# ErikNatanael/knaster

Measured on AMD Instinct MI355X. Metric: UGen-samples/sec (voices x block_size x UGens / s), higher is better.
Workload: dtype f32

## Files before the change

knaster_amd/csrc/voice_bank.hpp:

```cpp
#pragma once

namespace {

template <typename F>
struct Bank final : knh_bank {
  typedef typename knh_dev::WordOf<F>::type W;
  const knh::KernelEntry* entry = nullptr;
  const knh::PipeEntry* pipe = nullptr;
  bool pipe_pair = false;
  const knh::WideEntry* wide = nullptr;
  int wide_waves = 0;
  bool interp = false;
  std::vector<knh_dev::InterpOp> h_prog;
  knh_dev::InterpOp* d_prog = nullptr;
  unsigned interp_sigs = 0, interp_out = 0;
  const knh::JitKernel* frame_jit = nullptr;
  uint32_t* d_sin_slots = nullptr;
  unsigned frame_vpw = 1, n_sin = 0;
  uint64_t env_ranks = 0;
  const knh::JitKernel* jit = nullptr;
  int pipeline_level = 1;
  std::string signature;
  const char* debug_signature() const override { return signature.c_str(); }
  uint32_t nv = 0;
// ... 380 lines not shown
      const unsigned n_cuts = partition_chain(signature, cuts);
      jit = knh::jit_pipe_kernel(signature.c_str(), cuts, n_cuts, sizeof(F) == 8, desc.allow_fma != 0, &why);
      jit_pipe = jit != nullptr;
      if (!jit) return fail(why.rfind("JIT_CRASH: ", 0) == 0 ? KNH_ERR_INTERNAL : KNH_ERR_UNSUPPORTED_CHAIN, "run-time fusion of chain '" + signature + "' (pipelined) failed: " + why);
    } else if (!entry && !interp) {
      std::string why;
      unsigned jw = !signature_is_dag(signature) && n_groups > jit_pipe_max ? (n_groups <= 1024 ? 4u : 8u) : 1u;
      if (const char* e = std::getenv("KNH_JIT_WAVES")) { const int v = std::atoi(e); if ((v == 1 || v == 4 || v == 8 || v == 16) && !signature_is_dag(signature)) jw = static_cast<unsigned>(v); }
      if (sizeof(F) == 8 && jw == 16) jw = 8;
      jit = knh::jit_voice_kernel(signature.c_str(), sizeof(F) == 8, desc.allow_fma != 0, &why, jw);
      if (!jit) return fail(why.rfind("JIT_CRASH: ", 0) == 0 ? KNH_ERR_INTERNAL : KNH_ERR_UNSUPPORTED_CHAIN, "run-time fusion of chain '" + signature + "' failed: " + why);
    }
    sample_rate = sr;
    block_size = bs;
    stride = (static_cast<long>(nv) + 63) / 64 * 64;
    f2pi = 16384.0 * 65536.0 * (1.0 / static_cast<double>(sr));
    const F sr_as_f32 = static_cast<F>(static_cast<float>(sr));

    std::vector<W> st(static_cast<size_t>(n_slots) * stride, W(0));
    std::vector<double> seg_rows;
    auto slot = [&](int s, uint32_t v) -> W& { return st[static_cast<size_t>(s) * stride + v]; };
    auto fw = [](F x) { return static_cast<W>(to_bits(x)); };
    shadow.assign(stages.size(), Shadow{});
    for (size_t si = 0; si < stages.size(); ++si) {
      const StageInfo& S = stages[si];
      const double* ca = ctor[si].data();
      Shadow& sh = shadow[si];
      for (uint32_t v = 0; v < nv; ++v) {
        const double* a = ca + static_cast<size_t>(v) * S.n_ctor;
        switch (S.kind) {
          case KNH_STAGE_SIN_WT: {
            if (v == 0) sh.a.resize(nv);
            F freq = static_cast<F>(a[0]);
            sh.a[v] = freq;
            slot(S.slot_base + 0, v) = 0;
            slot(S.slot_base + 1, v) = 0;
            slot(S.slot_base + 2, v) = sat_u32(static_cast<double>(freq) * f2pi);
          } break;
          case KNH_STAGE_SIN_NUMERIC: {
            F freq = static_cast<F>(a[0]);
            slot(S.slot_base + 0, v) = fw(F(0));
            slot(S.slot_base + 1, v) = fw(F(0));
            slot(S.slot_base + 2, v) = fw(freq / sr_as_f32);
          } break;
          case KNH_STAGE_SVF: {
            if (v == 0) { sh.a.resize(nv); sh.b.resize(nv); sh.c.resize(nv); sh.ty.resize(nv); }
            double tyd = a[0];
            uint32_t ty = (tyd >= 0 && tyd <= 8) ? static_cast<uint32_t>(tyd) : 0u;
            sh.ty[v] = static_cast<uint8_t>(ty);
            sh.a[v] = static_cast<F>(a[1]); sh.b[v] = static_cast<F>(a[2]); sh.c[v] = static_cast<F>(a[3]);
            F co[6];
            svf_coeffs<F>(ty, sh.a[v], sh.b[v], sh.c[v], sr_as_f32, co);
            slot(S.slot_base + 0, v) = fw(F(0));
            slot(S.slot_base + 1, v) = fw(F(0));
            for (int k = 0; k < 6; ++k) slot(S.slot_base + 2 + k, v) = fw(co[k]);
            if (S.n_slots == 12) {
              slot(S.slot_base + 8, v) = fw(sh.a[v]); slot(S.slot_base + 9, v) = fw(sh.b[v]); slot(S.slot_base + 10, v) = fw(sh.c[v]);
              slot(S.slot_base + 11, v) = ty;
            }
          } break;
          case KNH_STAGE_ONEPOLE_LPF:
          case KNH_STAGE_ONEPOLE_HPF: {
            F freq = S.kind == KNH_STAGE_ONEPOLE_LPF ? static_cast<F>(a[0]) : F(0);
            F f = freq / sr_as_f32;
            F b1 = std::exp(F(-2.0) * Consts<F>::PI * f);
            F a0 = F(1.0) - b1;
            slot(S.slot_base + 0, v) = fw(F(0));
            slot(S.slot_base + 1, v) = fw(a0);
            slot(S.slot_base + 2, v) = fw(b1);
          } break;
          case KNH_STAGE_MUL_ENV_ASR:
          case KNH_STAGE_MUL_ENV_AR: {
            if (v == 0) { sh.a.resize(nv); sh.b.resize(nv); }
            F atk = static_cast<F>(a[0]), rel = static_cast<F>(a[1]);
            sh.a[v] = atk; sh.b[v] = rel;
            F ar = atk == F(0) ? F(1) : F(1) / (atk * static_cast<F>(sr));
            F rr = rel == F(0) ? F(1) : F(1) / (rel * static_cast<F>(sr));
// ... 1313 lines not shown
```

knaster_amd/csrc/voice_chain.hpp:

```cpp
#pragma once
#include "voice_stages.hpp"

namespace knh_dev {

template <typename F, bool FMA, int BASE, typename... S> struct Chain;
template <typename F, bool FMA, int BASE>
struct Chain<F, FMA, BASE> {
  static constexpr int kSlots = BASE;
  static constexpr bool kUsesSine = false;
  static constexpr bool kPan = false;
  static constexpr u64 kParamBits = 0ull, kNopOkBits = 0ull;
  static constexpr bool kBinds = false;
  static constexpr bool kUsesRing = false;
  template <int T> __device__ __forceinline__ void tick_tile_sw(const Chain&, u32, u64, F (&)[T], const Ctx&, u32) {}
  __device__ __forceinline__ void pan_gains(F&, F&) const {}
  template <typename W> __device__ __forceinline__ void load(const W*, long) {}
  template <typename W> __device__ __forceinline__ void store(W*, long) const {}
  __device__ __forceinline__ F tick(F x, const Ctx&, u32) { return x; }
  template <int T> __device__ __forceinline__ void tick_tile(F (&)[T], const Ctx&, u32) {}
#ifdef KNH_DAG_STAMPS
  template <int T> __device__ __forceinline__ void tick_tile_stamped(F (&)[T], const Ctx&, u32, u64*, u64&) {}
#endif
  __device__ __forceinline__ void on_event(u32, u32, u64, u32) {}
  __device__ __forceinline__ bool last_env_stopped(bool dflt) const { return dflt; }
  __device__ __forceinline__ u32 collect_done(u32 acc) const { return acc; }
  __device__ __forceinline__ void reset_marks() {}
  __device__ __forceinline__ void begin_block(u32, const Ctx&) {}
};
template <typename F, bool FMA, int BASE, typename S0, typename... Rest>
struct Chain<F, FMA, BASE, S0, Rest...> {
  typedef Chain<F, FMA, BASE + S0::kSlots, Rest...> RestT;
  static constexpr int kSlots = RestT::kSlots;
  static constexpr bool kUsesSine = S0::kUsesSine || RestT::kUsesSine;
  static constexpr bool kPan = IsPan<S0>::value || RestT::kPan;
  static constexpr u64 kStageBits = BASE + S0::kSlots <= 64 ? (((u64)1 << S0::kSlots) - 1) << (BASE < 64 ? BASE : 0) : 0ull;
  static constexpr u64 kParamBits = (BASE + S0::kSlots <= 64 ? (u64)S0::kParamMask << (BASE < 64 ? BASE : 0) : 0ull) | RestT::kParamBits;
  static constexpr u64 kNopOkBits = ((S0::kParamMask != 0u || !S0::kHasSeg) && BASE < 64 ? (u64)1 << (BASE < 64 ? BASE : 0) : 0ull) | RestT::kNopOkBits;
  static constexpr bool kBinds = S0::kNeedsBind || RestT::kBinds;
  static constexpr bool kUsesRing = S0::kUsesRing || RestT::kUsesRing;
  typename S0::template Regs<F> r;
  u32 mark = 0xFFFFFFFFu;
  RestT rest;
  template <typename W> __device__ __forceinline__ void load(const W* s, long stride) {
    S0::template load<F, W>(r, s + (long)BASE * stride, stride);
    rest.load(s, stride);
  }
  template <typename W> __device__ __forceinline__ void store(W* s, long stride) const {
    S0::template store<F, W>(r, s + (long)BASE * stride, stride);
    rest.store(s, stride);
  }
  __device__ __forceinline__ F tick(F x, const Ctx& c, u32 frame) {
    x = S0::template tick<F, FMA>(r, x, c, frame, mark);
    return rest.tick(x, c, frame);
  }
  template <int T> __device__ __forceinline__ void tick_tile(F (&x)[T], const Ctx& c, u32 frame0) {
    S0::template tick_tile<F, FMA, T>(r, x, c, frame0, mark);
    rest.template tick_tile<T>(x, c, frame0);
  }
#ifdef KNH_DAG_STAMPS
  template <int T> __device__ __forceinline__ void tick_tile_stamped(F (&x)[T], const Ctx& c, u32 frame0, u64* acc, u64& t_prev) {
    S0::template tick_tile<F, FMA, T>(r, x, c, frame0, mark);
    asm volatile("" : "+v"(x[T - 1]) : : "memory");
    const u64 t = __builtin_amdgcn_s_memtime();
    acc[0] += t - t_prev;
    t_prev = t;
    rest.template tick_tile_stamped<T>(x, c, frame0, acc + 1, t_prev);
  }
#endif
  template <int T> __device__ __forceinline__ void tick_tile_sw(const Chain& cn, u32 sw, u64 touched, F (&x)[T], const Ctx& c, u32 frame0) {
    bool hit = false;
    if constexpr (S0::kParamMask != 0u) hit = __builtin_amdgcn_ballot_w64((touched & kStageBits) != 0ull) != 0;
    if (hit) {
#pragma unroll
      for (int j = 0; j < T; ++j) {
        S0::take_params(r, cn.r, (u32)j == sw);
        x[j] = S0::template tick<F, FMA>(r, x[j], c, frame0 + j, mark);
      }
    } else {
#pragma unroll
      for (int j = 0; j < T; ++j) x[j] = S0::template tick<F, FMA>(r, x[j], c, frame0 + j, mark);
// ... 1031 lines not shown
```

knaster_amd/csrc/voice_pipe.hpp:

```cpp
#pragma once
#include "voice_chain.hpp"

namespace knh_dev {

template <typename... S> struct Group {};
template <int K, typename... S> struct Fan {};

template <typename G> struct GroupInfo;
template <typename... S> struct GroupInfo<Group<S...>> {
  static constexpr int slots = (0 + ... + S::kSlots);
  static constexpr bool uses_sine = (false || ... || S::kUsesSine);
  static constexpr bool uses_ring = (false || ... || S::kUsesRing);
  static constexpr bool has_env = (false || ... || S::kIsEnv);
  static constexpr bool pan = (false || ... || IsPan<S>::value);
  static constexpr int fan_for(int) { return 1; }
};
template <int K, typename... S> struct GroupInfo<Fan<K, S...>> {
  static constexpr int slots = (0 + ... + S::kSlots);
  static constexpr bool uses_sine = (false || ... || S::kUsesSine);
  static constexpr bool uses_ring = false;
  static constexpr bool has_env = false;
  static constexpr bool pan = false;
  static constexpr int fan_for(int T) { return K * 8 <= T ? K : (T >= 8 ? T / 8 : 1); }
  static_assert(((S::kMutableMask == 0u) && ...), "a Fan group's stages keep no state");
// ... 10 lines not shown
template <typename F> struct PipeTile {
  static constexpr int value = sizeof(F) == 4 ? 32 : 16;
  static constexpr int big = 2 * value;
};

template <typename F, int TILE> struct EdgeLayout {
  static constexpr int T = TILE;
  static constexpr int VW = 16 / (int)sizeof(F);
  static constexpr int stride = T + VW;
  static constexpr int tile = 64 * stride;
  typedef F Vec __attribute__((ext_vector_type(16 / sizeof(F))));
};
enum { PIPE_MIXER = 0, PIPE_FOLD = 1, PIPE_INPLACE = 2 };
template <int MODE, int NG> struct EdgeMap {
  static_assert(MODE != PIPE_INPLACE || NG >= 2, "an in-place last group reads an edge");
  static constexpr int tiles = MODE == PIPE_MIXER ? NG * 2 : NG * 2 - 1;
  static __device__ __forceinline__ int out_tile(int I, int g) {
    if (MODE == PIPE_FOLD && I == NG - 1) return I * 2;
    if (MODE == PIPE_INPLACE && I >= NG - 2) return (NG - 2) * 2 + g % 3;
    return I * 2 + (g & 1);
  }
  static __device__ __forceinline__ int in_tile(int I, int g) { return I > 0 ? out_tile(I - 1, g) : 0; }
  static __device__ __forceinline__ int mixer_tile(int g) { return out_tile(NG - 1, g); }
};
__device__ __forceinline__ void pipe_barrier() {
  __builtin_amdgcn_fence(__ATOMIC_RELEASE, "workgroup");
  __builtin_amdgcn_s_barrier();
  __builtin_amdgcn_fence(__ATOMIC_ACQUIRE, "workgroup");
}

template <typename F> struct PipeShared {
  float* sine;
  F* edge;
  const Event* ev_lds;
  u32 ev_lds_first, ev_lds_n;
  u32* res_slot;
  u32* res_marks;
  Event* ev_stage;
  u32 ev_cap, n_threads;
  __attribute__((address_space(3))) char* ring_tile_of[4];
};

template <typename F, bool FMA, int T, bool PAN>
__device__ __forceinline__ void pipe_fold_tile(const F* tile, const VoiceKernelArgs<F>& a, int lane, u32 wave_global, u32 n_waves_total,
                                               int blk, u32 n0, u32 len, u32 v0, u32 nv, u32 res_tile = 0u, u32 res_epoch = 0u);

// ... 93 lines not shown
    chain.reset_marks();
    const ResStaged st = res_stage_events(a.res, call, sh.ev_stage, sh.ev_cap, v0, nv, (u32)(wave_all * 64 + lane), sh.n_threads);
    ev_staged = st.count != 0u;
    ev_lds_first = st.first;
    ev_ranged = call.has_events && call.n_ranges != 0u;
    if (ev_ranged) { evs = nullptr; ev_i = 0; ev_end = call.n_ranges; }
  }
  if (!ev_ranged) {
    ev_i = 0; ev_end = 0;
    if (evs) {
      if (resident) { ev_i = *reinterpret_cast<const volatile u32*>(evs + voice); ev_end = *reinterpret_cast<const volatile u32*>(evs + voice + 1); }
      else { ev_i = evs[voice]; ev_end = evs[voice + 1]; }
    }
  }
  nxt.frame = 0xFFFFFFFFu; next_frame = 0xFFFFFFFFu;
  take_next();
  base = 0;

  const u32 n_frames = fend - fbeg;
  const int tpb = (int)((n_frames + T - 1) / T);
  const int n_tiles = tpb * (int)a.n_blocks;
  const int n_steps = n_tiles + NG - (MODE == PIPE_FOLD ? 1 : 0);
  const u32 n_waves_total = (a.n_voices + 63u) / 64u;
  int blk = 0, ti = 0;
#ifdef KNH_DAG_STAMPS
  u64 busy = 0, busy_in = 0, busy_out = 0, busy_tick = 0, busy_fold = 0;
#endif
  for (int s = 0; s < n_steps; ++s) {
    const int g = s - I;
    if (g >= 0 && g < n_tiles) {
#ifdef KNH_DAG_STAMPS
      const u64 t0 = __builtin_amdgcn_s_memtime();
#endif
      F x[TW];
      if (I > 0) {
        typedef typename EdgeLayout<F, T>::Vec Vec;
        constexpr int VW = EdgeLayout<F, T>::VW;
        const Vec* in = reinterpret_cast<const Vec*>(sh.edge + (long)Map::in_tile(I, g) * EdgeLayout<F, T>::tile +
                                                     (long)lane * EdgeLayout<F, T>::stride + fo);
#pragma unroll
        for (int j = 0; j < TW / VW; ++j) {
          const Vec v = in[j];
#pragma unroll
          for (int k = 0; k < VW; ++k) x[j * VW + k] = v[k];
        }
      } else {
#pragma unroll
        for (int j = 0; j < TW; ++j) x[j] = (F)0;
      }
      if (ti == 0) {
        ctx.input_block = reinterpret_cast<const F*>(a.input) + (long)blk * a.in_channels * a.block_size;
        chain.begin_block(fbeg, ctx);
      }
      const u32 n_tile = fbeg + (u32)ti * T;
      const u32 m_tile = fend - n_tile < (u32)T ? fend - n_tile : (u32)T;
      const u32 n = n_tile + fo;
      const u32 m = m_tile > fo ? (m_tile - fo < (u32)TW ? m_tile - fo : (u32)TW) : 0u;
      apply_events_upto(base + n);
      const bool ev_inside = next_frame < base + n + TW;
#if defined(KNH_DAG_STAMPS) || defined(KNH_TILE_FENCES)
      asm volatile("s_waitcnt lgkmcnt(0)" ::: "memory");
#endif
#ifdef KNH_DAG_STAMPS
      const u64 t1 = __builtin_amdgcn_s_memtime();
      busy_in += t1 - t0;
#endif
      {
        typedef typename EdgeLayout<F, T>::Vec Vec;
        constexpr int VW = EdgeLayout<F, T>::VW;
        F* out_tile = sh.edge + (long)Map::out_tile(I, g) * EdgeLayout<F, T>::tile;
        F* out_row = out_tile + (long)lane * EdgeLayout<F, T>::stride + fo;
        if (__builtin_expect(m == (u32)TW && !__builtin_amdgcn_ballot_w64(ev_inside), 1)) {
          chain.template tick_tile<TW>(x, ctx, n);
#ifdef KNH_DAG_STAMPS
          asm volatile("" ::: "memory");
          busy_tick += __builtin_amdgcn_s_memtime() - t1;
#endif
          Vec* out = reinterpret_cast<Vec*>(out_row);
#pragma unroll
          for (int j = 0; j < TW / VW; ++j) {
            Vec v;
#pragma unroll
            for (int k = 0; k < VW; ++k) v[k] = x[j * VW + k];
            out[j] = v;
          }
#ifdef KNH_AB_NO_SW
        } else if (false && [&]() -> bool {
#else
        } else if (m == (u32)TW && ChainT::kParamBits != 0ull && !ChainT::kBinds && [&]() -> bool {
#endif
          ChainT cn = chain;
          const u32 sv_i = ev_i;
          const Event sv_nxt = nxt;
          const u32 sv_next_frame = next_frame;
          const u32 tile_end = base + n + (u32)TW;
          u32 sw = (u32)TW;
          u64 touched = 0ull;
          bool bad = false;
          while (next_frame < tile_end) {
            const u32 op = nxt.slot_op >> 24, slot = nxt.slot_op & 0xFFFFFFu, code = op & 0x7Fu;
            if (slot >= SLOT_LO && slot < SLOT_HI) {
              const u32 rel = nxt.frame - (base + n);
              if (sw == (u32)TW) sw = rel;
              bad = bad || sw != rel || slot >= 64u ||
                    !((code == EV_SET && ((ChainT::kParamBits >> (slot & 63u)) & 1ull)) || (code == EV_NOP && ((ChainT::kNopOkBits >> (slot & 63u)) & 1ull)));
              if (!bad) {
                cn.on_event(op, slot, nxt.bits, nxt.frame - base);
                touched |= 1ull << (slot & 63u);
                if (live && code == EV_SET) a.state[(long)slot * a.stride + voice] = (W)nxt.bits;
              }
            }
            ++ev_i;
            take_next();
          }
          if (__builtin_amdgcn_ballot_w64(bad) != 0) {
            ev_i = sv_i;
            nxt = sv_nxt;
            next_frame = sv_next_frame;
            return false;
          }
          const F* in_row = sh.edge + (long)Map::in_tile(I, g) * EdgeLayout<F, T>::tile + (long)lane * EdgeLayout<F, T>::stride + fo;
          for (u32 j0 = 0; j0 < (u32)TW; j0 += 8u) {
            F sub[8];
            if (I > 0) {
#pragma unroll
              for (int q = 0; q < 8 / VW; ++q) {
                const Vec v = reinterpret_cast<const Vec*>(in_row + j0)[q];
#pragma unroll
                for (int k = 0; k < VW; ++k) sub[q * VW + k] = v[k];
              }
            } else {
#pragma unroll
              for (int k = 0; k < 8; ++k) sub[k] = (F)0;
            }
            chain.template tick_tile_sw<8>(cn, sw - j0, touched, sub, ctx, n + j0);
#pragma unroll
            for (int q = 0; q < 8 / VW; ++q) {
              Vec v;
#pragma unroll
              for (int k = 0; k < VW; ++k) v[k] = sub[q * VW + k];
              reinterpret_cast<Vec*>(out_row + j0)[q] = v;
            }
          }
          return true;
        }()) {
        } else {
          const F* in_row = sh.edge + (long)Map::in_tile(I, g) * EdgeLayout<F, T>::tile + (long)lane * EdgeLayout<F, T>::stride + fo;
          for (u32 j0 = 0; j0 < m; j0 += 8u) {
            const u32 cnt = m - j0 < 8u ? m - j0 : 8u;
            F sub[8];
            if (I > 0) {
#pragma unroll
              for (int q = 0; q < 8 / VW; ++q) {
                const Vec v = reinterpret_cast<const Vec*>(in_row + j0)[q];
#pragma unroll
                for (int k = 0; k < VW; ++k) sub[q * VW + k] = v[k];
              }
            } else {
#pragma unroll
              for (int k = 0; k < 8; ++k) sub[k] = (F)0;
            }
#pragma unroll
            for (int k = 0; k < 8; ++k) {
              if ((u32)k < cnt) {
                apply_events_upto(base + n + j0 + (u32)k);
                sub[k] = chain.tick(sub[k], ctx, n + j0 + (u32)k);
              }
            }
#pragma unroll
            for (int q = 0; q < 8 / VW; ++q) {
              Vec v;
#pragma unroll
              for (int k = 0; k < VW; ++k) v[k] = sub[q * VW + k];
              reinterpret_cast<Vec*>(out_row + j0)[q] = v;
            }
          }
        }
        if constexpr (GroupInfo<G>::pan) {
          F gl = (F)0, gr = (F)0;
          chain.pan_gains(gl, gr);
          out_row[T] = gl;
          out_row[T + 1] = gr;
        }
#ifdef KNH_DAG_STAMPS
        asm volatile("s_waitcnt lgkmcnt(0)" ::: "memory");
        const u64 tf0 = __builtin_amdgcn_s_memtime();
#endif
        if constexpr (FOLDS) pipe_fold_tile<F, FMA, T, GroupInfo<G>::pan>(out_tile, a, lane, wave_global, n_waves_total, blk, n_tile, m_tile, v0, nv);
#ifdef KNH_DAG_STAMPS
        asm volatile("s_waitcnt lgkmcnt(0)" ::: "memory");
        busy_fold += __builtin_amdgcn_s_memtime() - tf0;
#endif
      }
#if defined(KNH_DAG_STAMPS) || defined(KNH_TILE_FENCES)
      asm volatile("" ::: "memory");
#endif
#ifdef KNH_DAG_STAMPS
      const u64 t2 = __builtin_amdgcn_s_memtime();
#endif
      if (++ti == tpb) {
        apply_events_upto(base + fend);
        ti = 0;
        ++blk;
        base += a.block_size;
        if (resident) {
          sh.res_marks[wave_all * 64 + lane] = chain.collect_done(0xFFFFFFFFu);
          if (GroupInfo<G>::has_env && I == LAST_ENV) sh.res_marks[15 * 64 + lane] = live && !chain.last_env_stopped(false) ? 1u : 0u;
        }
      }
#if defined(KNH_DAG_STAMPS) || defined(KNH_TILE_FENCES)
      asm volatile("s_waitcnt lgkmcnt(0)" ::: "memory");
#endif
#ifdef KNH_DAG_STAMPS
      const u64 t3 = __builtin_amdgcn_s_memtime();
      busy += t3 - t0;
      busy_out += t3 - t2;
#endif
    }
    pipe_barrier();
  }
#ifdef KNH_DAG_STAMPS
  if (wave_global == 0u && lane == 0) {
    const u64 d = (u64)(n_tiles > 0 ? n_tiles : 1);
    a.flags[4 + I] = (u32)(busy / d);
    if (8 + 2 * I + 1 < 16) { a.flags[8 + 2 * I] = (u32)(busy_in / d); a.flags[9 + 2 * I] = (u32)(busy_out / d); }
    if (FOLDS) { a.flags[14] = (u32)(busy_tick / d); a.flags[15] = (u32)(busy_fold / d); }
    else if (MODE != PIPE_FOLD && I == 1) { a.flags[14] = (u32)(busy_tick / d); a.flags[15] = (u32)((busy - busy_in - busy_out - busy_tick) / d); }
  }
#endif
  done_frame = chain.collect_done(0xFFFFFFFFu);
  if (!resident) break;
  }
  if (live) chain.store(a.state + voice, a.stride);
  if (!resident && GroupInfo<G>::has_env && I == LAST_ENV) {
    const bool running = live && !chain.last_env_stopped(false);
    const u64 br = __builtin_amdgcn_ballot_w64(running);
    if (lane == 0 && br) atomicAdd(&a.flags[1], (u32)__builtin_popcountll(br));
  }
  return done_frame;
}

template <typename F, bool FMA, int T, bool PAN>
__device__ __forceinline__ void pipe_fold_tile(const F* tile, const VoiceKernelArgs<F>& a, int lane, u32 wave_global, u32 n_waves_total,
// ... 31 lines not shown
}

template <typename F, bool FMA, int T, int MODE, int NG, bool PAN, int CHAINW, bool HAS_ENV>
__device__ __forceinline__ void pipe_run_mixer(const PipeShared<F>& sh, const VoiceKernelArgs<F>& a, int lane, u32 wave_global,
                                               u32 v0, u32 nv, int wave_all) {
  u32 fbeg = a.frame_begin, fend = a.frame_end;
  const bool resident = a.res.bell != nullptr;
  u32 res_expect = a.res.first_epoch;
  const u32 n_waves_total = (a.n_voices + 63u) / 64u;
  for (;;) {
  ResCall call;
  call.epoch = 0u;
  if (resident) {
    call = res_wait(a.res, res_expect, sh.res_slot, wave_all, lane);
    if (call.leave) break;
    res_expect = (res_expect + 1u) & (u32)RES_EPOCH_MASK;
    fbeg = call.frame_begin;
    fend = call.frame_end;
    (void)res_stage_events(a.res, call, sh.ev_stage, sh.ev_cap, v0, nv, (u32)(wave_all * 64 + lane), sh.n_threads);
  }
  const u32 n_frames = fend - fbeg;
  const int tpb = (int)((n_frames + T - 1) / T);
  const int n_tiles = tpb * (int)a.n_blocks;
  const int n_steps = n_tiles + NG;
  int blk = 0, ti = 0;
#ifdef KNH_DAG_STAMPS
  u64 busy = 0;
#endif
  for (int s = 0; s < n_steps; ++s) {
    const int g = s - NG;
    if (g >= 0 && g < n_tiles) {
#ifdef KNH_DAG_STAMPS
      const u64 t0 = __builtin_amdgcn_s_memtime();
#endif
      const u32 rel = (u32)ti * T;
      const u32 len = n_frames - rel < (u32)T ? n_frames - rel : (u32)T;
      const F* tile = sh.edge + (long)EdgeMap<MODE, NG>::mixer_tile(g) * EdgeLayout<F, T>::tile;
      pipe_fold_tile<F, FMA, T, PAN>(tile, a, lane, wave_global, n_waves_total, blk, fbeg + rel, len, v0, nv, (u32)g, call.epoch);
      if (resident && g == n_tiles - 1) {
        u32 n_done = 0u, n_run = 0u;
        if (HAS_ENV) {
          u32 d = 0xFFFFFFFFu;
#pragma unroll
          for (int w = 0; w < CHAINW; ++w) d = sh.res_marks[w * 64 + lane] != 0xFFFFFFFFu ? sh.res_marks[w * 64 + lane] : d;
          const bool live = (u32)lane < nv;
          if (live) a.done_frames[v0 + lane] = d;
          n_done = (u32)__builtin_popcountll(__builtin_amdgcn_ballot_w64(live && d != 0xFFFFFFFFu));
          n_run = (u32)__builtin_popcountll(__builtin_amdgcn_ballot_w64(live && sh.res_marks[15 * 64 + lane] != 0u));
        }
        if (lane == 0) res_put(a.res.wg_flags + wave_global, n_done | (n_run << 8), res_tag(call.epoch, 255u));
      }
      if (++ti == tpb) { ti = 0; ++blk; }
#ifdef KNH_DAG_STAMPS
      asm volatile("s_waitcnt vmcnt(0) lgkmcnt(0)" ::: "memory");
      busy += __builtin_amdgcn_s_memtime() - t0;
#endif
    }
    if (resident) asm volatile("s_waitcnt lgkmcnt(0)\n\ts_barrier" ::: "memory");
    else pipe_barrier();
  }
#ifdef KNH_DAG_STAMPS
  if (wave_global == 0u && lane == 0) a.flags[4 + NG] = (u32)(busy / (u64)(n_tiles > 0 ? n_tiles : 1));
#endif
  if (!resident) break;
  }
}

template <typename F, bool FMA, int T, int MODE, int NG, int I, int BASE, int W0, int LAST_ENV, typename G, typename... Rest>
__device__ __forceinline__ u32 pipe_dispatch(int wave, const PipeShared<F>& sh, const VoiceKernelArgs<F>& a, int lane, u32 wave_global, u32 v0, u32 nv, int wave_all) {
  constexpr int KF = GroupInfo<G>::fan_for(T);
  if (wave >= W0 && wave < W0 + KF) return pipe_run_group<F, FMA, T, MODE, NG, I, BASE, LAST_ENV, G>(sh, a, lane, wave_global, v0, nv, wave - W0, wave_all);
  if constexpr (sizeof...(Rest) > 0)
    return pipe_dispatch<F, FMA, T, MODE, NG, I + 1, BASE + GroupInfo<G>::slots, W0 + KF, LAST_ENV, Rest...>(wave, sh, a, lane, wave_global, v0, nv, wave_all);
  return 0xFFFFFFFFu;
}
template <int T, int MODE, typename... Gs> struct PipeWaves {
  static constexpr int chain = (0 + ... + GroupInfo<Gs>::fan_for(T));
  static constexpr int value = chain + (MODE == PIPE_FOLD ? 0 : 1);
};

template <int I, typename... Gs> struct LastEnv;
template <int I> struct LastEnv<I> { static constexpr int value = -1; };
// ... 117 lines not shown
```

knaster_amd/csrc/voice_stages.hpp:

```cpp
#pragma once

extern "C" __device__ float __ocml_sin_f32(float);
extern "C" __device__ double __ocml_sin_f64(double);
extern "C" __device__ float __ocml_cos_f32(float);
extern "C" __device__ double __ocml_cos_f64(double);
extern "C" __device__ float __ocml_pow_f32(float, float);
extern "C" __device__ double __ocml_pow_f64(double, double);
extern "C" __device__ float __ocml_tan_f32(float);
extern "C" __device__ double __ocml_tan_f64(double);
extern "C" __device__ float __ocml_exp_f32(float);
extern "C" __device__ double __ocml_exp_f64(double);
extern "C" __device__ float __ocml_sqrt_f32(float);
extern "C" __device__ double __ocml_sqrt_f64(double);

namespace knh_dev {

typedef unsigned int u32;
typedef unsigned long long u64;

template <typename F> struct WordOf;
template <> struct WordOf<float> { typedef u32 type; };
template <> struct WordOf<double> { typedef u64 type; };

template <typename F> __device__ __forceinline__ F word_to_f(typename WordOf<F>::type w);
// ... 3 lines not shown
__device__ __forceinline__ u64 f_to_word(double f) { return __builtin_bit_cast(u64, f); }

template <bool FMA> __device__ __forceinline__ float mad(float a, float b, float c) {
  if constexpr (FMA) return __builtin_fmaf(a, b, c);
  else return a * b + c;
}
template <bool FMA> __device__ __forceinline__ double mad(double a, double b, double c) {
  if constexpr (FMA) return __builtin_fma(a, b, c);
  else return a * b + c;
}

__device__ __forceinline__ u32 sat_u32(double v) {
  u32 r;
  asm("v_cvt_u32_f64 %0, %1" : "=v"(r) : "v"(v));
  return r;
}

struct StageDefaults {
  static constexpr u32 kParamMask = 0u;
  template <typename R> static __device__ __forceinline__ void take_params(R&, const R&, bool) {}
  static constexpr bool kBinary = false;
  static constexpr int kArParam = -1;
  static constexpr bool kUsesRing = false;
};
template <typename S, int P> struct ArP : S {
  static constexpr int kArParam = P;
};

enum { EV_SET = 0, EV_ENV_ASR_RELEASE = 1, EV_NOP = 2, EV_SEGENV_STOP = 3, EV_ALLPASS_DELAY = 4, EV_SPLIT = 0x80  };

struct Event {
  u32 frame;
  u32 slot_op;
  u64 bits;
};

struct Ctx {
  const float* sine;
  double f2pi;
  const double* seg_table;
  u32 seg_max;
  void* delay_ring;
  u32 delay_stride;
  const void* buffer;
  const void* input_block;
  u32 in_stride;
// ... 838 lines not shown
      "v_pk_mul_f32 v[102:103], v[116:117], v[100:101] op_sel_hi:[1,0]\n\t"      \
      "v_pk_mul_f32 v[104:105], v[118:119], v[114:115] op_sel_hi:[1,0]\n\t"      \
      "v_add_f32 v103, v101, v103\n\t"                                       \
      "v_pk_add_f32 v[106:107], v[102:103], v[104:105]\n\t"                  \
      "v_mul_f32 v112, v122, %[x" #K "]\n\t"                                 \
      "v_pk_fma_f32 v[100:101], v[106:107], 2.0, v[100:101] op_sel_hi:[1,0,1] neg_lo:[0,0,1] neg_hi:[0,0,1]\n\t"    \
      "v_pk_mul_f32 v[108:109], v[120:121], v[106:107]\n\t"                  \
      KNH_SVF_WAIT                                                                                                     \
      "v_add_f32 v112, v112, v108\n\t"                                       \
      "v_add_f32 %[y" #K "], v112, v109\n\t"
#pragma unroll
    for (int j = 0; j < T; j += 8) {
      float y0, y1, y2, y3, y4, y5, y6, y7;
      asm volatile(KNH_SVF_STEP(0) KNH_SVF_STEP(1) KNH_SVF_STEP(2) KNH_SVF_STEP(3) KNH_SVF_STEP(4) KNH_SVF_STEP(5) KNH_SVF_STEP(6) KNH_SVF_STEP(7)
                   : [y0] "=&v"(y0), [y1] "=&v"(y1), [y2] "=&v"(y2), [y3] "=&v"(y3), [y4] "=&v"(y4), [y5] "=&v"(y5),
                     [y6] "=&v"(y6), [y7] "=&v"(y7), "+{v100}"(ic1), "+{v101}"(ic2)
                   : [x0] "v"(x[j]), [x1] "v"(x[j + 1]), [x2] "v"(x[j + 2]), [x3] "v"(x[j + 3]), [x4] "v"(x[j + 4]),
                     [x5] "v"(x[j + 5]), [x6] "v"(x[j + 6]), [x7] "v"(x[j + 7]), "{v116}"(a1), "{v117}"(a2), "{v118}"(a2b), "{v119}"(a3),
                     "{v120}"(m1), "{v121}"(m2), "{v122}"(m0)
                   : "v102", "v103", "v104", "v105", "v106", "v107", "v108", "v109", "v112", "v114", "v115");
      x[j] = y0; x[j + 1] = y1; x[j + 2] = y2; x[j + 3] = y3; x[j + 4] = y4; x[j + 5] = y5; x[j + 6] = y6; x[j + 7] = y7;
    }
#undef KNH_SVF_STEP
    r.ic1 = ic1; r.ic2 = ic2;
  }
  template <typename F> static __device__ __forceinline__ bool low_pass(const Regs<F>& r) {
    typedef typename WordOf<F>::type W;
    const W neg0 = (W)1 << (sizeof(F) * 8 - 1);
    const bool mine = r.nl == 0 && f_to_word(r.ic2) != neg0;
    return __builtin_amdgcn_ballot_w64(!mine) == 0;
  }
  template <int T>
  static __device__ __forceinline__ void tick_tile_low(Regs<float>& r, float (&x)[T]) {
    static_assert(T % 8 == 0, "the filter tile is unrolled in blocks of eight samples");
    float ic1 = r.ic1, ic2 = r.ic2;
    const float a1 = r.a1, a2 = r.a2, a2b = r.a2, a3 = r.a3;
#define KNH_SVF_LOW(K)                                                                                             \
      "v_sub_f32 v114, %[x" #K "], v101\n\t"                                 \
      "v_pk_mul_f32 v[102:103], v[116:117], v[100:101] op_sel_hi:[1,0]\n\t"      \
      "v_pk_mul_f32 v[104:105], v[118:119], v[114:115] op_sel_hi:[1,0]\n\t"      \
      "v_add_f32 v103, v101, v103\n\t"                                       \
      "v_pk_add_f32 v[106:107], v[102:103], v[104:105]\n\t"                  \
      KNH_SVF_WAIT                                                                                                     \
      "v_fma_f32 %[y" #K "], 0, v106, v107\n\t"                              \
      "v_pk_fma_f32 v[100:101], v[106:107], 2.0, v[100:101] op_sel_hi:[1,0,1] neg_lo:[0,0,1] neg_hi:[0,0,1]\n\t"    \
      KNH_SVF_WAIT
#pragma unroll
    for (int j = 0; j < T; j += 8) {
      float y0, y1, y2, y3, y4, y5, y6, y7;
      asm volatile(KNH_SVF_LOW(0) KNH_SVF_LOW(1) KNH_SVF_LOW(2) KNH_SVF_LOW(3) KNH_SVF_LOW(4) KNH_SVF_LOW(5) KNH_SVF_LOW(6) KNH_SVF_LOW(7)
                   : [y0] "=&v"(y0), [y1] "=&v"(y1), [y2] "=&v"(y2), [y3] "=&v"(y3), [y4] "=&v"(y4), [y5] "=&v"(y5),
                     [y6] "=&v"(y6), [y7] "=&v"(y7), "+{v100}"(ic1), "+{v101}"(ic2)
                   : [x0] "v"(x[j]), [x1] "v"(x[j + 1]), [x2] "v"(x[j + 2]), [x3] "v"(x[j + 3]), [x4] "v"(x[j + 4]),
                     [x5] "v"(x[j + 5]), [x6] "v"(x[j + 6]), [x7] "v"(x[j + 7]), "{v116}"(a1), "{v117}"(a2), "{v118}"(a2b), "{v119}"(a3)
                   : "v102", "v103", "v104", "v105", "v106", "v107", "v114", "v115");
      x[j] = y0; x[j + 1] = y1; x[j + 2] = y2; x[j + 3] = y3; x[j + 4] = y4; x[j + 5] = y5; x[j + 6] = y6; x[j + 7] = y7;
    }
#undef KNH_SVF_LOW
    r.ic1 = ic1; r.ic2 = ic2;
  }
  template <int T>
  static __device__ __forceinline__ void tick_tile_low_f64(Regs<double>& r, double (&x)[T]) {
    double ic1 = r.ic1, ic2 = r.ic2;
    const double a1 = r.a1, a2 = r.a2, a3 = r.a3;
    double v1p = 0.0, v2p = 0.0;
#define KNH_STEP(stmt) stmt; __builtin_amdgcn_sched_barrier(0)
#pragma unroll
    for (int j = 0; j < T; ++j) {
      KNH_STEP(const double v3 = x[j] - ic2);
      KNH_STEP(const double p2 = a2 * ic1);
      KNH_STEP(const double p1 = a1 * ic1);
      KNH_STEP(const double q2 = a3 * v3);
      KNH_STEP(const double q1 = a2 * v3);
      KNH_STEP(const double t = ic2 + p2);
      if (j > 0) { KNH_STEP(x[j - 1] = __builtin_fma(0.0, v1p, v2p)); }
      KNH_STEP(const double v2 = t + q2);
      KNH_STEP(const double v1 = p1 + q1);
      KNH_STEP(ic2 = __builtin_fma(2.0, v2, -ic2));
      KNH_STEP(ic1 = __builtin_fma(2.0, v1, -ic1));
      v1p = v1; v2p = v2;
    }
    x[T - 1] = __builtin_fma(0.0, v1p, v2p);
// ... 10 lines not shown
    for (int j = 0; j < T; ++j) {
      double o1 = 0.0, o2 = 0.0, s = 0.0;
      KNH_STEP(const double v3 = x[j] - ic2);
      KNH_STEP(const double p1 = a1 * ic1);
      KNH_STEP(const double p2 = a2 * ic1);
      if (j > 0) { KNH_STEP(o1 = m1 * v1p); }
      KNH_STEP(const double q1 = a2 * v3);
      KNH_STEP(const double q2 = a3 * v3);
      KNH_STEP(const double t = ic2 + p2);
      if (j > 0) { KNH_STEP(o2 = m2 * v2p); }
      KNH_STEP(const double v1 = p1 + q1);
      KNH_STEP(const double v2 = t + q2);
      if (j > 0) { KNH_STEP(s = o0p + o1); }
      KNH_STEP(ic1 = __builtin_fma(2.0, v1, -ic1));
      KNH_STEP(ic2 = __builtin_fma(2.0, v2, -ic2));
      KNH_STEP(const double o0 = m0 * x[j]);
      if (j > 0) { KNH_STEP(x[j - 1] = s + o2); }
      v1p = v1; v2p = v2; o0p = o0;
    }
    x[T - 1] = (o0p + m1 * v1p) + m2 * v2p;
#undef KNH_STEP
    r.ic1 = ic1; r.ic2 = ic2;
  }
  template <typename F, bool FMA, int T>
  static __device__ __forceinline__ void tick_tile(Regs<F>& r, F (&x)[T], const Ctx& c, u32 frame0, u32& done_frame) {
    if constexpr (sizeof(F) == 4 && !FMA) {
      if (low_pass(r)) tick_tile_low<T>(r, x); else tick_tile_packed<T>(r, x);
    } else if constexpr (sizeof(F) == 8 && !FMA) {
      if (low_pass(r)) tick_tile_low_f64<T>(r, x); else tick_tile_f64<T>(r, x);
    } else {
#pragma unroll
      for (int j = 0; j < T; ++j) x[j] = tick<F, FMA>(r, x[j], c, frame0 + j, done_frame);
    }
  }
  template <typename F>
  static __device__ __forceinline__ void on_event(Regs<F>& r, u32 op, u32 rel, u64 bits, u32 ) {
    if ((op & 0x7Fu) != EV_SET) return;
    F v = word_to_f<F>((typename WordOf<F>::type)bits);
    r.ic1 = rel == 0 ? v : r.ic1; r.ic2 = rel == 1 ? v : r.ic2; r.a1 = rel == 2 ? v : r.a1; r.a2 = rel == 3 ? v : r.a2;
    r.a3 = rel == 4 ? v : r.a3; r.m0 = rel == 5 ? v : r.m0; r.m1 = rel == 6 ? v : r.m1; r.m2 = rel >= 7 ? v : r.m2;
    note_mix(r);
  }
};

static __device__ __forceinline__ float dev_pow(float a, float b) { return __ocml_pow_f32(a, b); }
static __device__ __forceinline__ double dev_pow(double a, double b) { return __ocml_pow_f64(a, b); }
struct SvfP : Svf {
  static constexpr int kSlots = 12;
  static constexpr u32 kParamMask = 0u;
  template <typename F> struct Regs : Svf::Regs<F> { F cutoff, q, gain; u32 ty; };
  template <typename F, typename W>
  static __device__ __forceinline__ void load(Regs<F>& r, const W* s, long st) {
    Svf::load<F, W>(r, s, st);
    r.cutoff = word_to_f<F>(s[8 * st]); r.q = word_to_f<F>(s[9 * st]); r.gain = word_to_f<F>(s[10 * st]); r.ty = (u32)s[11 * st];
  }
  template <typename F, typename W>
  static __device__ __forceinline__ void store(const Regs<F>& r, W* s, long st) {
    Svf::store<F, W>(r, s, st);
    s[2 * st] = f_to_word(r.a1); s[3 * st] = f_to_word(r.a2); s[4 * st] = f_to_word(r.a3);
    s[5 * st] = f_to_word(r.m0); s[6 * st] = f_to_word(r.m1); s[7 * st] = f_to_word(r.m2);
    s[8 * st] = f_to_word(r.cutoff); s[9 * st] = f_to_word(r.q); s[10 * st] = f_to_word(r.gain);
  }
  static __device__ __forceinline__ float tan_f(float v) { return __ocml_tan_f32(v); }
  static __device__ __forceinline__ double tan_f(double v) { return __ocml_tan_f64(v); }
  static __device__ __forceinline__ float sqrt_f(float v) { return __ocml_sqrt_f32(v); }
  static __device__ __forceinline__ double sqrt_f(double v) { return __ocml_sqrt_f64(v); }
  template <typename F>
  static __device__ __forceinline__ void set_coeffs(Regs<F>& r, const Ctx& c) {
    const F one = (F)1, sr = (F)(float)c.sample_rate;
    F g = tan_f(((F)3.14159265358979323846 * r.cutoff) / sr);
    F k = one / r.q;
    F m0 = (F)0, m1 = (F)0, m2 = (F)0, amp = (F)0;
// ... 978 lines not shown
```

Measured before the change: 2924 billion.

## Run event-free tile streaks in pipe kernel with hoisted SVF mode check

Restructures the pipelined voice kernel loop from a per-step dispatch into per-block loops. An inner fast path processes consecutive full tiles without events, using incrementally advanced edge tile indices instead of recomputing the tile map each step. A RunPrep mechanism evaluates the SVF low-pass mode check once per run rather than once per tile, and the mixer loop gets a similar incremental tile index. It also adds odd pinned-register inline asm for the SVF state writeback and a debug env toggle that seeds -0.0 into SVF state, which may constrain register allocation.

```diff
diff --git a/knaster_amd/csrc/voice_bank.hpp b/knaster_amd/csrc/voice_bank.hpp
--- a/knaster_amd/csrc/voice_bank.hpp
+++ b/knaster_amd/csrc/voice_bank.hpp
@@ -426,6 +426,8 @@
     auto slot = [&](int s, uint32_t v) -> W& { return st[static_cast<size_t>(s) * stride + v]; };
     auto fw = [](F x) { return static_cast<W>(to_bits(x)); };
     shadow.assign(stages.size(), Shadow{});
+    const char* const neg0_env = std::getenv("KNH_DEBUG_SVF_IC2_NEG0");
+    const bool svf_ic2_neg0 = neg0_env && neg0_env[0] == '1';
     for (size_t si = 0; si < stages.size(); ++si) {
       const StageInfo& S = stages[si];
       const double* ca = ctor[si].data();
@@ -456,7 +458,7 @@
             F co[6];
             svf_coeffs<F>(ty, sh.a[v], sh.b[v], sh.c[v], sr_as_f32, co);
             slot(S.slot_base + 0, v) = fw(F(0));
-            slot(S.slot_base + 1, v) = fw(F(0));
+            slot(S.slot_base + 1, v) = fw(svf_ic2_neg0 && v % 3 == 0 ? F(-0.0) : F(0));
             for (int k = 0; k < 6; ++k) slot(S.slot_base + 2 + k, v) = fw(co[k]);
             if (S.n_slots == 12) {
               slot(S.slot_base + 8, v) = fw(sh.a[v]); slot(S.slot_base + 9, v) = fw(sh.b[v]); slot(S.slot_base + 10, v) = fw(sh.c[v]);
diff --git a/knaster_amd/csrc/voice_chain.hpp b/knaster_amd/csrc/voice_chain.hpp
--- a/knaster_amd/csrc/voice_chain.hpp
+++ b/knaster_amd/csrc/voice_chain.hpp
@@ -18,6 +18,9 @@
   template <typename W> __device__ __forceinline__ void store(W*, long) const {}
   __device__ __forceinline__ F tick(F x, const Ctx&, u32) { return x; }
   template <int T> __device__ __forceinline__ void tick_tile(F (&)[T], const Ctx&, u32) {}
+  struct RunPrep {};
+  __device__ __forceinline__ RunPrep prepare_run() const { return RunPrep(); }
+  template <int T> __device__ __forceinline__ void tick_tile_run(F (&)[T], const Ctx&, u32, const RunPrep&) {}
 #ifdef KNH_DAG_STAMPS
   template <int T> __device__ __forceinline__ void tick_tile_stamped(F (&)[T], const Ctx&, u32, u64*, u64&) {}
 #endif
@@ -56,6 +59,19 @@
   template <int T> __device__ __forceinline__ void tick_tile(F (&x)[T], const Ctx& c, u32 frame0) {
     S0::template tick_tile<F, FMA, T>(r, x, c, frame0, mark);
     rest.template tick_tile<T>(x, c, frame0);
+  }
+  struct RunPrep { bool mine; typename RestT::RunPrep rest; };
+  __device__ __forceinline__ RunPrep prepare_run() const {
+    RunPrep p;
+    if constexpr (S0::kHasRunPrep) p.mine = S0::template prepare_run<F>(r);
+    else p.mine = false;
+    p.rest = rest.prepare_run();
+    return p;
+  }
+  template <int T> __device__ __forceinline__ void tick_tile_run(F (&x)[T], const Ctx& c, u32 frame0, const RunPrep& p) {
+    if constexpr (S0::kHasRunPrep) S0::template tick_tile_prepared<F, FMA, T>(r, x, c, frame0, mark, p.mine);
+    else S0::template tick_tile<F, FMA, T>(r, x, c, frame0, mark);
+    rest.template tick_tile_run<T>(x, c, frame0, p.rest);
   }
 #ifdef KNH_DAG_STAMPS
   template <int T> __device__ __forceinline__ void tick_tile_stamped(F (&x)[T], const Ctx& c, u32 frame0, u64* acc, u64& t_prev) {
diff --git a/knaster_amd/csrc/voice_pipe.hpp b/knaster_amd/csrc/voice_pipe.hpp
--- a/knaster_amd/csrc/voice_pipe.hpp
+++ b/knaster_amd/csrc/voice_pipe.hpp
@@ -56,6 +56,13 @@
   }
   static __device__ __forceinline__ int in_tile(int I, int g) { return I > 0 ? out_tile(I - 1, g) : 0; }
   static __device__ __forceinline__ int mixer_tile(int g) { return out_tile(NG - 1, g); }
+  static __device__ __forceinline__ int next_out(int I, int t) {
+    if (MODE == PIPE_FOLD && I == NG - 1) return t;
+    if (MODE == PIPE_INPLACE && I >= NG - 2) return t == (NG - 2) * 2 + 2 ? (NG - 2) * 2 : t + 1;
+    return t ^ 1;
+  }
+  static __device__ __forceinline__ int next_in(int I, int t) { return I > 0 ? next_out(I - 1, t) : 0; }
+  static __device__ __forceinline__ int next_mixer(int t) { return next_out(NG - 1, t); }
 };
 __device__ __forceinline__ void pipe_barrier() {
   __builtin_amdgcn_fence(__ATOMIC_RELEASE, "workgroup");
@@ -195,60 +202,61 @@
   const int n_tiles = tpb * (int)a.n_blocks;
   const int n_steps = n_tiles + NG - (MODE == PIPE_FOLD ? 1 : 0);
   const u32 n_waves_total = (a.n_voices + 63u) / 64u;
-  int blk = 0, ti = 0;
+  const int full = n_frames >= fo + (u32)TW ? (int)((n_frames - fo - (u32)TW) / (u32)T) + 1 : 0;
+  int in_t = Map::in_tile(I, 0), out_t = Map::out_tile(I, 0);
 #ifdef KNH_DAG_STAMPS
   u64 busy = 0, busy_in = 0, busy_out = 0, busy_tick = 0, busy_fold = 0;
 #endif
-  for (int s = 0; s < n_steps; ++s) {
-    const int g = s - I;
-    if (g >= 0 && g < n_tiles) {
+  for (int s = 0; s < I; ++s) pipe_barrier();
+  for (int blk = 0, ti = 0; blk < (tpb > 0 ? (int)a.n_blocks : 0); ++blk) {
+    ctx.input_block = reinterpret_cast<const F*>(a.input) + (long)blk * a.in_channels * a.block_size;
+    chain.begin_block(fbeg, ctx);
+    for (ti = 0;;) {
+      typedef typename EdgeLayout<F, T>::Vec Vec;
+      constexpr int VW = EdgeLayout<F, T>::VW;
 #ifdef KNH_DAG_STAMPS
       const u64 t0 = __builtin_amdgcn_s_memtime();
 #endif
-      F x[TW];
-      if (I > 0) {
-        typedef typename EdgeLayout<F, T>::Vec Vec;
-        constexpr int VW = EdgeLayout<F, T>::VW;
-        const Vec* in = reinterpret_cast<const Vec*>(sh.edge + (long)Map::in_tile(I, g) * EdgeLayout<F, T>::tile +
-                                                     (long)lane * EdgeLayout<F, T>::stride + fo);
-#pragma unroll
-        for (int j = 0; j < TW / VW; ++j) {
-          const Vec v = in[j];
-#pragma unroll
-          for (int k = 0; k < VW; ++k) x[j * VW + k] = v[k];
-        }
-      } else {
-#pragma unroll
-        for (int j = 0; j < TW; ++j) x[j] = (F)0;
-      }
-      if (ti == 0) {
-        ctx.input_block = reinterpret_cast<const F*>(a.input) + (long)blk * a.in_channels * a.block_size;
-        chain.begin_block(fbeg, ctx);
-      }
       const u32 n_tile = fbeg + (u32)ti * T;
-      const u32 m_tile = fend - n_tile < (u32)T ? fend - n_tile : (u32)T;
       const u32 n = n_tile + fo;
-      const u32 m = m_tile > fo ? (m_tile - fo < (u32)TW ? m_tile - fo : (u32)TW) : 0u;
       apply_events_upto(base + n);
       const bool ev_inside = next_frame < base + n + TW;
+      bool step_open = true;
+      if (__builtin_expect(ti < full && !__builtin_amdgcn_ballot_w64(ev_inside), 1)) {
+        const typename ChainT::RunPrep prep = chain.prepare_run();
+        u32 nq = n;
+        for (;;) {
+#ifdef KNH_DAG_STAMPS
+          const u64 q0 = __builtin_amdgcn_s_memtime();
+#endif
+          F x[TW];
+          if (I > 0) {
+            const Vec* in = reinterpret_cast<const Vec*>(sh.edge + (long)in_t * EdgeLayout<F, T>::tile + (long)lane * EdgeLayout<F, T>::stride + fo);
+#pragma unroll
+            for (int j = 0; j < TW / VW; ++j) {
+              const Vec v = in[j];
+#pragma unroll
+              for (int k = 0; k < VW; ++k) x[j * VW + k] = v[k];
+            }
+          } else {
+#pragma unroll
+            for (int j = 0; j < TW; ++j) x[j] = (F)0;
+          }
 #if defined(KNH_DAG_STAMPS) || defined(KNH_TILE_FENCES)
-      asm volatile("s_waitcnt lgkmcnt(0)" ::: "memory");
-#endif
-#ifdef KNH_DAG_STAMPS
-      const u64 t1 = __builtin_amdgcn_s_memtime();
-      busy_in += t1 - t0;
-#endif
-      {
-        typedef typename EdgeLayout<F, T>::Vec Vec;
-        constexpr int VW = EdgeLayout<F, T>::VW;
-        F* out_tile = sh.edge + (long)Map::out_tile(I, g) * EdgeLayout<F, T>::tile;
-        F* out_row = out_tile + (long)lane * EdgeLayout<F, T>::stride + fo;
-        if (__builtin_expect(m == (u32)TW && !__builtin_amdgcn_ballot_w64(ev_inside), 1)) {
-          chain.template tick_tile<TW>(x, ctx, n);
+          asm volatile("s_waitcnt lgkmcnt(0)" ::: "memory");
+#endif
+#ifdef KNH_DAG_STAMPS
+          const u64 q1 = __builtin_amdgcn_s_memtime();
+          busy_in += q1 - q0;
+#endif
+          chain.template tick_tile_run<TW>(x, ctx, nq, prep);
 #ifdef KNH_DAG_STAMPS
           asm volatile("" ::: "memory");
-          busy_tick += __builtin_amdgcn_s_memtime() - t1;
-#endif
+          const u64 q2 = __builtin_amdgcn_s_memtime();
+          busy_tick += q2 - q1;
+#endif
+          F* const out_tile = sh.edge + (long)out_t * EdgeLayout<F, T>::tile;
+          F* const out_row = out_tile + (long)lane * EdgeLayout<F, T>::stride + fo;
           Vec* out = reinterpret_cast<Vec*>(out_row);
 #pragma unroll
           for (int j = 0; j < TW / VW; ++j) {
@@ -257,10 +265,48 @@
             for (int k = 0; k < VW; ++k) v[k] = x[j * VW + k];
             out[j] = v;
           }
+          if constexpr (GroupInfo<G>::pan) {
+            F gl = (F)0, gr = (F)0;
+            chain.pan_gains(gl, gr);
+            out_row[T] = gl;
+            out_row[T + 1] = gr;
+          }
+#ifdef KNH_DAG_STAMPS
+          asm volatile("s_waitcnt lgkmcnt(0)" ::: "memory");
+          const u64 qf = __builtin_amdgcn_s_memtime();
+#endif
+          if constexpr (FOLDS) pipe_fold_tile<F, FMA, T, GroupInfo<G>::pan>(out_tile, a, lane, wave_global, n_waves_total, blk, nq, (u32)T, v0, nv);
+#ifdef KNH_DAG_STAMPS
+          asm volatile("s_waitcnt lgkmcnt(0)" ::: "memory");
+          const u64 qe = __builtin_amdgcn_s_memtime();
+          busy_fold += qe - qf;
+#endif
+          in_t = Map::next_in(I, in_t);
+          out_t = Map::next_out(I, out_t);
+          nq += (u32)T;
+          ++ti;
+#if defined(KNH_DAG_STAMPS) || defined(KNH_TILE_FENCES)
+          asm volatile("s_waitcnt lgkmcnt(0)" ::: "memory");
+#endif
+#ifdef KNH_DAG_STAMPS
+          const u64 q3 = __builtin_amdgcn_s_memtime();
+          busy_out += q3 - qe;
+          busy += q3 - q0;
+#endif
+          if (ti >= full) break;
+          pipe_barrier();
+          if (__builtin_amdgcn_ballot_w64(next_frame < base + nq + TW)) { step_open = false; break; }
+        }
+      } else {
+        const u32 m_tile = fend - n_tile < (u32)T ? fend - n_tile : (u32)T;
+        const u32 m = m_tile > fo ? (m_tile - fo < (u32)TW ? m_tile - fo : (u32)TW) : 0u;
+        F* const out_tile = sh.edge + (long)out_t * EdgeLayout<F, T>::tile;
+        F* const out_row = out_tile + (long)lane * EdgeLayout<F, T>::stride + fo;
+        const F* const in_row = sh.edge + (long)in_t * EdgeLayout<F, T>::tile + (long)lane * EdgeLayout<F, T>::stride + fo;
 #ifdef KNH_AB_NO_SW
-        } else if (false && [&]() -> bool {
+        if (false && [&]() -> bool {
 #else
-        } else if (m == (u32)TW && ChainT::kParamBits != 0ull && !ChainT::kBinds && [&]() -> bool {
+        if (m == (u32)TW && ChainT::kParamBits != 0ull && !ChainT::kBinds && [&]() -> bool {
 #endif
           ChainT cn = chain;
           const u32 sv_i = ev_i;
@@ -292,7 +338,6 @@
             next_frame = sv_next_frame;
             return false;
           }
-          const F* in_row = sh.edge + (long)Map::in_tile(I, g) * EdgeLayout<F, T>::tile + (long)lane * EdgeLayout<F, T>::stride + fo;
           for (u32 j0 = 0; j0 < (u32)TW; j0 += 8u) {
             F sub[8];
             if (I > 0) {
@@ -318,7 +363,6 @@
           return true;
         }()) {
         } else {
-          const F* in_row = sh.edge + (long)Map::in_tile(I, g) * EdgeLayout<F, T>::tile + (long)lane * EdgeLayout<F, T>::stride + fo;
           for (u32 j0 = 0; j0 < m; j0 += 8u) {
             const u32 cnt = m - j0 < 8u ? m - j0 : 8u;
             F sub[8];
@@ -360,38 +404,33 @@
         const u64 tf0 = __builtin_amdgcn_s_memtime();
 #endif
         if constexpr (FOLDS) pipe_fold_tile<F, FMA, T, GroupInfo<G>::pan>(out_tile, a, lane, wave_global, n_waves_total, blk, n_tile, m_tile, v0, nv);
+        in_t = Map::next_in(I, in_t);
+        out_t = Map::next_out(I, out_t);
+        ++ti;
 #ifdef KNH_DAG_STAMPS
         asm volatile("s_waitcnt lgkmcnt(0)" ::: "memory");
-        busy_fold += __builtin_amdgcn_s_memtime() - tf0;
+        const u64 t3 = __builtin_amdgcn_s_memtime();
+        busy_fold += t3 - tf0;
+        busy += t3 - t0;
 #endif
       }
-#if defined(KNH_DAG_STAMPS) || defined(KNH_TILE_FENCES)
-      asm volatile("" ::: "memory");
-#endif
-#ifdef KNH_DAG_STAMPS
-      const u64 t2 = __builtin_amdgcn_s_memtime();
-#endif
-      if (++ti == tpb) {
+      if (ti == tpb) {
         apply_events_upto(base + fend);
-        ti = 0;
-        ++blk;
         base += a.block_size;
         if (resident) {
           sh.res_marks[wave_all * 64 + lane] = chain.collect_done(0xFFFFFFFFu);
           if (GroupInfo<G>::has_env && I == LAST_ENV) sh.res_marks[15 * 64 + lane] = live && !chain.last_env_stopped(false) ? 1u : 0u;
         }
+#if defined(KNH_DAG_STAMPS) || defined(KNH_TILE_FENCES)
+        asm volatile("s_waitcnt lgkmcnt(0)" ::: "memory");
+#endif
+        pipe_barrier();
+        break;
       }
-#if defined(KNH_DAG_STAMPS) || defined(KNH_TILE_FENCES)
-      asm volatile("s_waitcnt lgkmcnt(0)" ::: "memory");
-#endif
-#ifdef KNH_DAG_STAMPS
-      const u64 t3 = __builtin_amdgcn_s_memtime();
-      busy += t3 - t0;
-      busy_out += t3 - t2;
-#endif
-    }
-    pipe_barrier();
-  }
+      if (step_open) pipe_barrier();
+    }
+  }
+  for (int s = I + n_tiles; s < n_steps; ++s) pipe_barrier();
 #ifdef KNH_DAG_STAMPS
   if (wave_global == 0u && lane == 0) {
     const u64 d = (u64)(n_tiles > 0 ? n_tiles : 1);
@@ -469,20 +508,23 @@
   const u32 n_frames = fend - fbeg;
   const int tpb = (int)((n_frames + T - 1) / T);
   const int n_tiles = tpb * (int)a.n_blocks;
-  const int n_steps = n_tiles + NG;
-  int blk = 0, ti = 0;
 #ifdef KNH_DAG_STAMPS
   u64 busy = 0;
 #endif
-  for (int s = 0; s < n_steps; ++s) {
-    const int g = s - NG;
-    if (g >= 0 && g < n_tiles) {
+  auto step_barrier = [&]() {
+    if (resident) asm volatile("s_waitcnt lgkmcnt(0)\n\ts_barrier" ::: "memory");
+    else pipe_barrier();
+  };
+  for (int s = 0; s < NG; ++s) step_barrier();
+  int mix_t = EdgeMap<MODE, NG>::mixer_tile(0);
+  int g = 0;
+  for (int blk = 0; blk < (tpb > 0 ? (int)a.n_blocks : 0); ++blk) {
+    for (u32 rel = 0; rel < n_frames; rel += (u32)T) {
 #ifdef KNH_DAG_STAMPS
       const u64 t0 = __builtin_amdgcn_s_memtime();
 #endif
-      const u32 rel = (u32)ti * T;
       const u32 len = n_frames - rel < (u32)T ? n_frames - rel : (u32)T;
-      const F* tile = sh.edge + (long)EdgeMap<MODE, NG>::mixer_tile(g) * EdgeLayout<F, T>::tile;
+      const F* tile = sh.edge + (long)mix_t * EdgeLayout<F, T>::tile;
       pipe_fold_tile<F, FMA, T, PAN>(tile, a, lane, wave_global, n_waves_total, blk, fbeg + rel, len, v0, nv, (u32)g, call.epoch);
       if (resident && g == n_tiles - 1) {
         u32 n_done = 0u, n_run = 0u;
@@ -497,14 +539,14 @@
         }
         if (lane == 0) res_put(a.res.wg_flags + wave_global, n_done | (n_run << 8), res_tag(call.epoch, 255u));
       }
-      if (++ti == tpb) { ti = 0; ++blk; }
+      mix_t = EdgeMap<MODE, NG>::next_mixer(mix_t);
+      ++g;
 #ifdef KNH_DAG_STAMPS
       asm volatile("s_waitcnt vmcnt(0) lgkmcnt(0)" ::: "memory");
       busy += __builtin_amdgcn_s_memtime() - t0;
 #endif
-    }
-    if (resident) asm volatile("s_waitcnt lgkmcnt(0)\n\ts_barrier" ::: "memory");
-    else pipe_barrier();
+      step_barrier();
+    }
   }
 #ifdef KNH_DAG_STAMPS
   if (wave_global == 0u && lane == 0) a.flags[4 + NG] = (u32)(busy / (u64)(n_tiles > 0 ? n_tiles : 1));
diff --git a/knaster_amd/csrc/voice_stages.hpp b/knaster_amd/csrc/voice_stages.hpp
--- a/knaster_amd/csrc/voice_stages.hpp
+++ b/knaster_amd/csrc/voice_stages.hpp
@@ -49,6 +49,7 @@
   static constexpr bool kBinary = false;
   static constexpr int kArParam = -1;
   static constexpr bool kUsesRing = false;
+  static constexpr bool kHasRunPrep = false;
 };
 template <typename S, int P> struct ArP : S {
   static constexpr int kArParam = P;
@@ -933,7 +934,9 @@
       x[j] = y0; x[j + 1] = y1; x[j + 2] = y2; x[j + 3] = y3; x[j + 4] = y4; x[j + 5] = y5; x[j + 6] = y6; x[j + 7] = y7;
     }
 #undef KNH_SVF_STEP
-    r.ic1 = ic1; r.ic2 = ic2;
+    float o1, o2;
+    asm volatile("v_mov_b32 %0, v100\n\tv_mov_b32 %1, v101" : "=&v"(o1), "=&v"(o2) : "{v100}"(ic1), "{v101}"(ic2));
+    r.ic1 = o1; r.ic2 = o2;
   }
   template <typename F> static __device__ __forceinline__ bool low_pass(const Regs<F>& r) {
     typedef typename WordOf<F>::type W;
@@ -968,7 +971,9 @@
       x[j] = y0; x[j + 1] = y1; x[j + 2] = y2; x[j + 3] = y3; x[j + 4] = y4; x[j + 5] = y5; x[j + 6] = y6; x[j + 7] = y7;
     }
 #undef KNH_SVF_LOW
-    r.ic1 = ic1; r.ic2 = ic2;
+    float o1, o2;
+    asm volatile("v_mov_b32 %0, v100\n\tv_mov_b32 %1, v101" : "=&v"(o1), "=&v"(o2) : "{v100}"(ic1), "{v101}"(ic2));
+    r.ic1 = o1; r.ic2 = o2;
   }
   template <int T>
   static __device__ __forceinline__ void tick_tile_low_f64(Regs<double>& r, double (&x)[T]) {
@@ -1025,16 +1030,22 @@
 #undef KNH_STEP
     r.ic1 = ic1; r.ic2 = ic2;
   }
+  static constexpr bool kHasRunPrep = true;
+  template <typename F> static __device__ __forceinline__ bool prepare_run(const Regs<F>& r) { return low_pass(r); }
+  template <typename F, bool FMA, int T>
+  static __device__ __forceinline__ void tick_tile_prepared(Regs<F>& r, F (&x)[T], const Ctx& c, u32 frame0, u32& done_frame, bool low) {
+    if constexpr (sizeof(F) == 4 && !FMA) {
+      if (low) tick_tile_low<T>(r, x); else tick_tile_packed<T>(r, x);
+    } else if constexpr (sizeof(F) == 8 && !FMA) {
+      if (low) tick_tile_low_f64<T>(r, x); else tick_tile_f64<T>(r, x);
+    } else {
+#pragma unroll
+      for (int j = 0; j < T; ++j) x[j] = tick<F, FMA>(r, x[j], c, frame0 + j, done_frame);
+    }
+  }
   template <typename F, bool FMA, int T>
   static __device__ __forceinline__ void tick_tile(Regs<F>& r, F (&x)[T], const Ctx& c, u32 frame0, u32& done_frame) {
-    if constexpr (sizeof(F) == 4 && !FMA) {
-      if (low_pass(r)) tick_tile_low<T>(r, x); else tick_tile_packed<T>(r, x);
-    } else if constexpr (sizeof(F) == 8 && !FMA) {
-      if (low_pass(r)) tick_tile_low_f64<T>(r, x); else tick_tile_f64<T>(r, x);
-    } else {
-#pragma unroll
-      for (int j = 0; j < T; ++j) x[j] = tick<F, FMA>(r, x[j], c, frame0 + j, done_frame);
-    }
+    tick_tile_prepared<F, FMA, T>(r, x, c, frame0, done_frame, low_pass(r));
   }
   template <typename F>
   static __device__ __forceinline__ void on_event(Regs<F>& r, u32 op, u32 rel, u64 bits, u32 ) {
@@ -1051,6 +1062,7 @@
 struct SvfP : Svf {
   static constexpr int kSlots = 12;
   static constexpr u32 kParamMask = 0u;
+  static constexpr bool kHasRunPrep = false;
   template <typename F> struct Regs : Svf::Regs<F> { F cutoff, q, gain; u32 ty; };
   template <typename F, typename W>
   static __device__ __forceinline__ void load(Regs<F>& r, const W* s, long st) {
```

Result: faster. 3223 billion, median of 6 (+10.2%).
